# sergioacg/Model-Predictive-Control-Tuning

Hardware: AMD Instinct MI355X
Metric: closed-loop GPC sims/sec (Shell 3x3, N2=30 Nu=5) over tuning grid (higher is better)
Workload: dtype f64; 1 GPU; Shell3x3 GAM scoring: 4096 candidates/GPU x nit=500 closed loop + J1 + RCCL all-gather + ranking; candidates_per_gpu=4096, N2=30, Nu=5, nit=500, parallelism=dp1

## Files before the change

model-predictive-control-tuning_amd/csrc/gpc_kernel.hip:

```cpp
#include <hip/hip_runtime.h>
#include <math.h>

#include "mpct_dev.h"
#include "gi_core.h"
#include "gpc_qp.h"
#include "gpc_qp16.h"
#include "gpc_prologue.h"
#include "gpc_record.h"

namespace mpct {

constexpr int kWaves16 = 3;

struct LdsLayout {
  int rinv, jt, dv, ra, sl, gb, A, x, xc, uprev, yprev, ucum, ye, yeh, uring, mzh, smz, frh, plb, pla, mzb,
      mza, frb, fra, total;
};

__host__ __device__ inline LdsLayout lds_layout(const DevScenario& sc, int M, bool ext) {
  const int nx = sc.nx, nu = sc.nu, nin = sc.nin, ne = sc.ne, my = sc.my;
  const int nmz = sc.dtc ? 2 * my * nu : 0;
  const int nfr = sc.dtc ? my : 0;
  const int ncp = ext ? 2 : 1;
  LdsLayout L;
// ... 428 lines not shown
      st | (nf ? MPCT_ST_NONFINITE_ : 0), iters);
}

}

#include <string>

#include "work_order.h"
#include "launch_fan.h"

namespace mpct {

long long small_lds_bytes(const DevScenario& sc, int M);
int launch_small(const DevScenario& sc, long long C, int nref, const int* N2, const int* Nu, const double* delta,
                 const double* lambda, const double* r, const DevOpts& o, const DevResult& out, const int* perm,
                 int first, hipStream_t stream, std::string* err);
long long dtc_small_lds_bytes(const DevScenario& sc, int M);
int launch_dtc_small(const DevScenario& sc, int cls, long long C, int nref, const int* N2, const int* Nu,
                     const double* delta, const double* lambda, const double* r, const double* v, const DevOpts& o,
                     const DevResult& out, const int* perm, int mlo, int first, hipStream_t stream, std::string* err);

long long lds_bytes_for(const DevScenario& sc, int N2, int Nu, bool ext) {
  (void)N2;
  const int M = sc.nu * Nu;
  if (sc.small && !ext && M <= 16) return small_lds_bytes(sc, M);
  if (sc.small_dtc && !ext && M <= 32) return dtc_small_lds_bytes(sc, M);
  LdsLayout L = lds_layout(sc, M, ext);
  return (long long)L.total * 8;
}

template <int MAXM>
// ... 42 lines not shown
    if (cls <= 32 && sc.small_dtc && !ext) {
      nm += (nm.empty() ? "" : " + ") + std::string("dtc_small_kernel<") + std::to_string(cls) + ">";
      continue;
    }
    if (nm.empty()) nm = "gpc_closed_loop_kernel<" + std::to_string(cls) + tail;
    else if (nm.find("gpc_closed_loop_kernel") == std::string::npos)
      nm += " + gpc_closed_loop_kernel<" + std::to_string(cls) + tail;
    else nm += " + <" + std::to_string(cls) + tail;
  }
  return nm;
}

int launch_closed_loop(const DevScenario& sc, long long C, int nref, const int* N2, const int* Nu,
                       const double* delta, const double* lambda, const double* r,
                       const double* v, const DevOpts& o, const DevResult& out, int maxM,
                       WorkOrder* wo, LaunchFan* fan, hipStream_t stream, std::string* err) {
  if (maxM > 64) {
    *err = "nu*nu_max > 64";
    return -4;
  }
  const int* perm = nullptr;
  DevResult lo = out;
  bool prefilled = false;
  if (wo) {
    if (C >= kOrderMinC) {
      lo.srow = stage_row(out, sc.my, sc.nu);
      const int rs = lo.srow.w ? order_stage(*wo, C * nref, lo.srow.w, &lo.stage, err) : 0;
      if (rs) return rs;
    }
    const int rc = order_candidates(kOrderGpc, sc.my, sc.nu, C, N2, Nu, delta, lambda, *wo, &perm, stream, err,
                                    &sc, nref, r, &lo, &prefilled);
    if (rc) return rc;
  }
  if (!perm) {
    lo = out;
    prefilled = false;
  }
  int rc = prefilled ? 0 : prefill_results(lo, C * nref, sc.my, sc.nu, stream, err);
  if (rc) return rc;
  FanScope fs(top_class(maxM) > 16 ? fan : nullptr, stream);
  int k = 0, mlo = 0;
  for (int cls = 16; cls <= top_class(maxM) && rc == 0; cls *= 2) {
    if (sc.nu > cls) {
      mlo = cls;
      continue;
    }
    const hipStream_t st = fs.stream(k);
    const int first = k == 0;
    const bool ext = o.open_loop || o.want_traj;
    if (diag_drop_launch(k)) rc = 0;
    else if (cls == 16 && sc.small && !ext) rc = launch_small(sc, C, nref, N2, Nu, delta, lambda, r, o, lo, perm, first, st, err);
    else if (cls <= 32 && sc.small_dtc && !ext)
      rc = launch_dtc_small(sc, cls, C, nref, N2, Nu, delta, lambda, r, v, o, lo, perm, mlo, first, st, err);
    else if (cls == 16) rc = launch_t<16>(sc, C, nref, N2, Nu, delta, lambda, r, v, o, lo, perm, mlo, first, st, err);
    else if (cls == 32) rc = launch_t<32>(sc, C, nref, N2, Nu, delta, lambda, r, v, o, lo, perm, mlo, first, st, err);
    else rc = launch_t<64>(sc, C, nref, N2, Nu, delta, lambda, r, v, o, lo, perm, mlo, first, st, err);
    mlo = cls;
    ++k;
  }
  fs.join();
  if (rc == 0 && lo.stage) rc = unpermute_results(*wo, C, nref, sc.my, sc.nu, lo.srow, out, stream, err);
  if (perm) order_mark_used(*wo, stream);
  return rc;
}

}
// ... 1 lines not shown
```

model-predictive-control-tuning_amd/csrc/gpc_qp16.h:

```cpp
#pragma once
#include "gi_core.h"

namespace mpct {

typedef double d4v[4];
#define FOR4(r, ...)             \
  do {                           \
    { constexpr int r = 0; __VA_ARGS__ } \
    { constexpr int r = 1; __VA_ARGS__ } \
    { constexpr int r = 2; __VA_ARGS__ } \
    { constexpr int r = 3; __VA_ARGS__ } \
  } while (0)

struct RegFactors {
  d4v J;
  double* sB;
};
constexpr int kBS = 16;


__device__ __forceinline__ int qlane() {
  int l = threadIdx.x;
  asm volatile("" : "+v"(l));
  return l;
}
__device__ __forceinline__ int q16_i() { return qlane() & 15; }
__device__ __forceinline__ int q16_b() { return qlane() >> 4; }

__device__ __forceinline__ double sel4u_v(double x0, double x1, double x2, double x3, int r) {
  double v = x0;
  if (r == 1) v = x1;
  if (r == 2) v = x2;
  if (r == 3) v = x3;
  return v;
}
#define sel4u(x, r) sel4u_v((x)[0], (x)[1], (x)[2], (x)[3], (r))
__device__ __forceinline__ double sel4v_v(double x0, double x1, double x2, double x3, int r) {
  const double lo = (r & 1) ? x1 : x0;
  const double hi = (r & 1) ? x3 : x2;
  return (r & 2) ? hi : lo;
}
#define sel4v(x, r) sel4v_v((x)[0], (x)[1], (x)[2], (x)[3], (r))

__device__ __forceinline__ void row16_sum4(d4v& t) {
  FOR4(r, t[r] += dppd<kQx1>(t[r]););
  FOR4(r, t[r] += dppd<kQx2>(t[r]););
  FOR4(r, t[r] += dppd<kHalfMirror>(t[r]););
  FOR4(r, t[r] += dppd<kMirror>(t[r]););
}

__device__ __forceinline__ double cvec_at(const d4v& c, int k) {
  return bcast(sel4u(c, k & 3), (k >> 2) * 16);
}

__device__ __forceinline__ void b_row4(const double* sB, d4v& x) {
  const double2* p = reinterpret_cast<const double2*>(sB + q16_i() * kBS + 4 * q16_b());
  const double2 u = p[0], v = p[1];
  x[0] = u.x;
  x[1] = u.y;
  x[2] = v.x;
  x[3] = v.y;
}

__device__ __forceinline__ double rows_down(double v) { return __shfl(v, qlane() + 16, 64); }
__device__ __forceinline__ double rows_up(double v) { return __shfl(v, qlane() - 16, 64); }

__device__ __forceinline__ void rot_pair(double& a, double& c, bool on, double cs, double sn) {
  if (on) {
    const double a0 = a, c0 = c;
    a = cs * a0 + sn * c0;
    c = -sn * a0 + cs * c0;
  }
}
__device__ __forceinline__ void rb_rotate_cols(d4v& x, int jj, double cs, double sn) {
  const int b = q16_b(), b0 = jj >> 2;
  const bool on = b == b0;
  switch (jj & 3) {
    case 0: {
      double a = x[0], c = x[1];
      rot_pair(a, c, on, cs, sn);
      x[0] = a;
      x[1] = c;
      break;
    }
    case 1: {
      double a = x[1], c = x[2];
      rot_pair(a, c, on, cs, sn);
      x[1] = a;
      x[2] = c;
      break;
    }
    case 2: {
      double a = x[2], c = x[3];
      rot_pair(a, c, on, cs, sn);
      x[2] = a;
      x[3] = c;
      break;
    }
    default: {
      const double nx0 = rows_down(x[0]), pv3 = rows_up(x[3]);
      if (on) x[3] = cs * x[3] + sn * nx0;
      if (b == b0 + 1) x[0] = -sn * pv3 + cs * x[0];
      break;
    }
  }
}

struct BoxMark16 {
  template <class St>
  __device__ __forceinline__ void operator()(St& S, int p, bool on) const {
    if (q16_i() == (p >> 2)) {
      if (on) S.act |= 1u << (p & 3);
      else S.act &= ~(1u << (p & 3));
    }
  }
};

template <bool PACKED>
__device__ __forceinline__ int rinv_idx(int i, int k, int M) {
  return PACKED ? i * M - ((i * (i - 1)) >> 1) + (k - i) : i * M + k;
}

template <bool PACKED>
__device__ __forceinline__ void gi16_load_rinv(GIState<16>& S, RegFactors& F, const double* sRi, int M) {
  const int i = q16_i(), b = q16_b();
  FOR4(r, {
    const int k = 4 * b + r;
    F.J[r] = (i < M && k < M && k >= i) ? sRi[rinv_idx<PACKED>(i, k, M)] : 0.0;
  });
  if (i < M) {
    double2* p = reinterpret_cast<double2*>(F.sB + i * kBS + 4 * b);
    p[0] = make_double2(0.0, 0.0);
    p[1] = make_double2(0.0, 0.0);
  }
  S.nrot = 0;
  S.jinit = true;
}

__device__ __forceinline__ void gi16_dvec(const RegFactors& F, int j0, int mp, double sg, d4v& d) {
  const int i = q16_i();
  if (j0 == mp) {
    const int src = j0 + 16 * q16_b();
    FOR4(r, d[r] = __shfl(F.J[r], src, kWave););
  } else {
    const bool in = i >= j0 && i <= mp;
    FOR4(r, d[r] = in ? F.J[r] : 0.0;);
    row16_sum4(d);
  }
  FOR4(r, d[r] *= sg;);
}

__device__ __forceinline__ void gi16_products(const RegFactors& F, const d4v& Bl, const d4v& d, int q,
                                              double& z, double& jq, double& rk, double& dn2, double& beta) {
  const int b = q16_b();
  double za = 0.0, ra = 0.0, s1 = 0.0, s2 = 0.0;
  FOR4(r, {
    const bool tail = 4 * b + r >= q;
    const double d2 = d[r] * d[r];
    s1 += d2;
    if (tail) {
      za = fma(F.J[r], d[r], za);
      s2 += d2;
    } else {
      ra = fma(Bl[r], d[r], ra);
    }
  });
  const double jl = (b == (q >> 2)) ? sel4u(F.J, q & 3) : 0.0;
  z = za;
  jq = jl;
  rk = ra;
  dn2 = s1;
  row4_sum4(z, jq, rk, dn2);
  beta = row4_sum(s2);
}

template <class Mark>
__device__ __forceinline__ void gi16_add(GIState<16>& S, RegFactors& F, double* sRA, int M, int p,
                                         const d4v& d, double beta, double z, double jq, double rk,
                                         double upm, const Mark& mark) {
  const int lane = qlane(), i = lane & 15, b = lane >> 4;
  const int q = S.q;
  const double dq = cvec_at(d, q);
  const double nrm = beta * rsq_nr(beta);
  const double alpha = dq > 0.0 ? -nrm : nrm;
  const double vq = dq - alpha;
  const double two_vtv = qp_rcp(beta - alpha * dq);
  const double f = (z - alpha * jq) * two_vtv;
  const double ia = qp_rcp(alpha);
  FOR4(r, {
    const int k = 4 * b + r;
    if (k >= q) F.J[r] = fma(-f, k == q ? vq : d[r], F.J[r]);
  });
  if (lane <= q) F.sB[lane * kBS + q] = lane < q ? -rk * ia : ia;
  if (lane < q) F.sB[q * kBS + lane] = 0.0;
  {
    const int w = 4 * b + i;
    if (i < 4 && w < q) sRA[w * M + q] = sel4v(d, i);
    if (lane == 0) sRA[q * M + q] = alpha;
  }
  if (i == q) {
    S.uw = upm;
    S.ww = p;
  }
  mark(S, p, true);
  S.q = q + 1;
  S.nrot += 1;
  lds_sync();
}

template <class Mark>
__device__ __forceinline__ void gi16_drop(GIState<16>& S, RegFactors& F, double* sRA, int M, int kd,
                                          const Mark& mark) {
  const int lane = qlane(), i = lane & 15;
  const int q = S.q;
  double* sB = F.sB;
  const int idk = __builtin_amdgcn_readlane(S.ww, kd);
  mark(S, idk, false);
  lds_sync();
  if (lane < q) {
    for (int w = kd; w < q - 1; ++w) {
      sRA[lane * M + w] = sRA[lane * M + w + 1];
      sB[w * kBS + lane] = sB[(w + 1) * kBS + lane];
    }
  }
  {
    const double un = lane_next<16>(S.uw);
    const int wn = lane_next_i<16>(S.ww);
    if (i >= kd && i < q - 1) {
// ... 7 lines not shown
    const double a = sRA[jj * M + jj], c = sRA[(jj + 1) * M + jj];
    const double rr = a * a + c * c;
    if (rr != 0.0) {
      const double ri = rsq_nr(rr);
      const double cs = a * ri, sn = c * ri;
      if (lane >= jj && lane < q - 1) {
        const double r0 = sRA[jj * M + lane], r1 = sRA[(jj + 1) * M + lane];
        sRA[jj * M + lane] = cs * r0 + sn * r1;
        sRA[(jj + 1) * M + lane] = (lane == jj) ? 0.0 : -sn * r0 + cs * r1;
      }
      if (lane < q) {
        const double b0 = sB[lane * kBS + jj], b1 = sB[lane * kBS + jj + 1];
        sB[lane * kBS + jj] = cs * b0 + sn * b1;
        sB[lane * kBS + jj + 1] = -sn * b0 + cs * b1;
      }
      rb_rotate_cols(F.J, jj, cs, sn);
      S.nrot += 1;
    }
    lds_sync();
  }
  const int qn = q - 1;
  if (i == qn) {
    S.uw = 0.0;
    S.ww = -1;
  }
  S.q = qn;
  lds_sync();
}

template <bool PACKED = false, class PAcc = void, bool BLDS = false>
__device__ __forceinline__ int gi_qp16(const double* sRi, double* sRA, int M, int Nu,
                                       const RowCons& rc, double up_row, double xu, double tol, int maxit,
                                       int* st, GIState<16>& S, RegFactors& F, int rebuild, double& xout
#ifdef MPCT_PROFILE
                                       , PAcc& pacc, unsigned long long& pprev
#endif
                                       ) {
  const int lane = qlane(), i = lane & 15;
  const bool row = i < M;
  if (!row) up_row = 0.0;
  const int rl = rc.l;
  double lo_box = 0.0, hi_box = 0.0;
  if constexpr (!BLDS) {
    lo_box = fmax(rc.dmin, rc.umin - up_row);
    hi_box = fmin(rc.dmax, rc.umax - up_row);
  }
  auto slacks = [&](double x, double s[4]) {
    double dmin, dmax, umin, umax, lo, hi;
    if constexpr (BLDS) {
      const double2 a = reinterpret_cast<const double2*>(rc.bnd)[0], b = reinterpret_cast<const double2*>(rc.bnd)[1];
      dmin = a.x;
      dmax = a.y;
      umin = b.x;
// ... 10 lines not shown
    }
    const double pre = block_prefix<16>(x, rl, Nu, row, nullptr);
    if (rl == 0) {
      s[0] = x - lo;
      s[1] = hi - x;
      s[2] = INFINITY;
      s[3] = INFINITY;
    } else {
      s[0] = x - dmin;
      s[1] = dmax - x;
      s[2] = pre - (umin - up_row);
      s[3] = (umax - up_row) - pre;
    }
    if (!row) s[0] = s[1] = s[2] = s[3] = INFINITY;
  };
  const BoxMark16 mark{};
  auto add = [&](int p, const d4v& d, double beta, double z, double jq, double rk, double upm)
                 __attribute__((always_inline)) { gi16_add(S, F, sRA, M, p, d, beta, z, jq, rk, upm, mark); };
  int it = 0;
  double xm = xu;
  PSTAMP(PROF_QCHECK);
  {
    double s[4];
    slacks(xu, s);
    const double smin = fmin(fmin(s[0], s[1]), fmin(s[2], s[3]));
    if (__ballot(smin < -tol) == 0) {
      xout = xu;
      return 0;
    }
    PSTAMP(PROF_QWENTRY);
    if (S.q == 0) {
      S.jinit = false;
    } else {
      if (!S.jinit || S.nrot >= rebuild * M) {
        const int qq = S.q;
#ifdef MPCT_PROFILE
        pacc[PROF_QWREADD] += (unsigned long long)qq * kProfCount;
#endif
        gi16_load_rinv<PACKED>(S, F, sRi, M);
        S.q = 0;
        for (int v = 0; v < qq; ++v) {
          const int p = __builtin_amdgcn_readlane(S.ww, v);
          int j0, mp;
          double sg;
          gi_normal(p, rc, j0, mp, sg);
          d4v Bl, d;
          lds_sync();
          b_row4(F.sB, Bl);
          gi16_dvec(F, j0, mp, sg, d);
          double z, jq, rk, dn2, beta;
          gi16_products(F, Bl, d, v, z, jq, rk, dn2, beta);
          const double uk = S.uw;
          add(p, d, beta, z, jq, rk, 0.0);
          if (i == v) S.uw = uk;
          ++it;
        }
        S.nrot = 0;
      }
      PSTAMP(PROF_QWREB);
      lds_sync();
      double c;
      {
        const int src = (S.ww >= 0 ? S.ww >> 2 : 0) + 16 * q16_b();
        const double g0 = __shfl(s[0], src, kWave), g1 = __shfl(s[1], src, kWave);
        const double g2 = __shfl(s[2], src, kWave), g3 = __shfl(s[3], src, kWave);
        c = i < S.q ? -sel4v_v(g0, g1, g2, g3, S.ww & 3) : 0.0;
      }
      PSTAMP(PROF_QWGATH);
      for (;;) {
        const int q = S.q;
        if (q == 0) {
          xm = xu;
          break;
        }
        d4v Bl, w;
        b_row4(F.sB, Bl);
        FOR4(r, w[r] = i < q ? Bl[r] * c : 0.0;);
        row16_sum4(w);
        const int b = q16_b();
        double xa = 0.0, la = 0.0;
        FOR4(r, {
          if (4 * b + r < q) {
            xa = fma(F.J[r], w[r], xa);
            la = fma(Bl[r], w[r], la);
          }
        });
        row4_sum2(xa, la);
        xm = xu + xa;
        const double lam = la;
        if (i < q) S.uw = lam;
        double lmin = i < q ? lam : INFINITY;
        int kd = i;
        qargmin<16>(lmin, kd, 0);
        PSTAMP(PROF_QWSOLVE);
        if (!(lmin < 0.0)) break;
#ifdef MPCT_PROFILE
        pacc[PROF_QWROT] += (unsigned long long)(S.q - 1 - kd) * kProfCount;
#endif
#ifdef MPCT_DIAG
        if (!(S.diag & kDiagSkipWarmDrop))
#endif
        {
          gi16_drop(S, F, sRA, M, kd, mark);
          {
            const double cn = lane_next<16>(c);
            if (i >= kd && i < q - 1) c = cn;
            else if (i == q - 1) c = 0.0;
          }
        }
        PSTAMP(PROF_QWDROP);
        if (++it >= maxit) {
          *st |= MPCT_ST_QP_MAXITER_;
          break;
        }
      }
      if (!row) xm = 0.0;
    }
  }
// ... 6 lines not shown
      slacks(xm, s);
#pragma unroll
      for (int k = 0; k < 4; ++k)
        if (!((S.act >> k) & 1u) && s[k] < best) {
          best = s[k];
          bid = 4 * i + k;
        }
    }
    qargmin<16>(best, bid, 2);
    PSTAMP(PROF_QCHECK);
    if (!(best < -tol)) break;
    if (it >= maxit) {
      *st |= MPCT_ST_QP_MAXITER_;
      break;
    }
    if (!S.jinit) gi16_load_rinv<PACKED>(S, F, sRi, M);
    const int p = bid;
    int j0, mp;
    double sgp;
    gi_normal(p, rc, j0, mp, sgp);
    double sp = best;
    double upm = 0.0;
    bool infeas = false;
    for (;;) {
      ++it;
      d4v Bl, d;
      b_row4(F.sB, Bl);
      gi16_dvec(F, j0, mp, sgp, d);
      double zm, jq, rk, dn2, beta;
      gi16_products(F, Bl, d, S.q, zm, jq, rk, dn2, beta);
      PSTAMP(PROF_QD);
      double t1 = INFINITY;
      int kdrop = 0x7fffffff;
      if (i < S.q && rk > 0.0) {
        t1 = qp_div(S.uw, rk);
        kdrop = i;
      }
      qargmin<16>(t1, kdrop, 0);
      const double t2 = (beta > 1e-14 * dn2) ? -qp_div(sp, beta) : INFINITY;
      const bool t2inf = __builtin_amdgcn_readfirstlane((int)(t2 == INFINITY)) != 0;
      if (t1 == INFINITY && t2inf) {
        *st |= MPCT_ST_QP_INFEAS_;
        infeas = true;
        break;
      }
// ... 5 lines not shown
      sp += t * beta;
      PSTAMP(PROF_QR);
      if (full) {
        add(p, d, beta, zm, jq, rk, upm);
        PSTAMP(PROF_QADD);
        break;
      }
      if (kdrop >= S.q) {
        *st |= MPCT_ST_NONFINITE_;
        infeas = true;
        break;
      }
#ifdef MPCT_PROFILE
      pacc[PROF_QROT] += (unsigned long long)(S.q - 1 - kdrop) * kProfCount;
#endif
      gi16_drop(S, F, sRA, M, kdrop, mark);
      PSTAMP(PROF_QDROP);
      if (it >= maxit) {
        *st |= MPCT_ST_QP_MAXITER_;
        break;
      }
    }
    if (infeas) break;
  }
  xout = xm;
  return it;
}

}
```

model-predictive-control-tuning_amd/csrc/gpc_small.hip:

```cpp
#include <hip/hip_runtime.h>
#include <math.h>

#include "mpct_dev.h"
#include "gi_core.h"
#include "gpc_qp.h"
#include "gpc_qp16.h"
#include "gpc_prologue.h"
#include "gpc_record.h"

namespace mpct {

struct SmallLayout {
  int rinv, ra, gb, A, xy, ring, hist, bnd, total;
};
__host__ __device__ inline SmallLayout small_layout(const DevScenario& sc, int M) {
  SmallLayout L;
  int o = 0;
  auto take = [&](int n) { int r = o; o += (n + 1) & ~1; return r; };
  L.rinv = take(M * (M + 1) / 2);
  L.ra = take(M * M);
  L.gb = take(M * kBS);
  L.A = take(M * kSmA);
  L.xy = take(kSmY);
  L.ring = take(3 * 2 * kSmR);
  L.hist = take(kSmEOff + 4 * sc.my * sc.sm_ke);
  L.bnd = take(4 * 3);
  L.total = (o + 1) & ~1;
  return L;
}

__device__ __forceinline__ int sm_lane() {
  int l = threadIdx.x;
  asm volatile("" : "+v"(l));
  return l;
}

__global__ void __launch_bounds__(64, 4)
    gpc_small_kernel(const DevScenario sc, long long C, int nref, const int* __restrict__ N2v,
                     const int* __restrict__ Nuv, const double* __restrict__ deltav,
                     const double* __restrict__ lambdav, const double* __restrict__ rv,
                     const int* __restrict__ perm, const DevOpts o, const DevResult out, int first) {
  extern __shared__ __attribute__((aligned(16))) double lds[];
  const int lane = threadIdx.x;
  const long long slot = blockIdx.x;
  const long long S = C * nref;
  if (slot >= S) return;
  const long long cs = slot / nref;
  const int kref = (int)(slot - cs * nref);
  const long long c = perm ? (long long)perm[cs] : cs;
  const long long sim = c * nref + kref;
  const int my = sc.my, nu = sc.nu, nit = sc.nit;
  const int N2 = N2v[c], Nu = Nuv[c];
  const int M = nu * Nu;
  auto write_nan = [&](int status) __attribute__((always_inline)) {
    put_record(out, slot, S, sim, my, nu, lane, NAN, NAN, NAN, NAN, status, 0);
  };
  if (N2 <= 0) {
    if (first) write_nan(MPCT_ST_SKIPPED_);
    return;
  }
  if (N2 > sc.n2max || Nu < 1 || Nu > sc.numax || Nu > N2) {
    if (first) write_nan(MPCT_ST_BADHORIZON_);
    return;
  }
  if (M > 16) return;
// ... 20 lines not shown
  const double pcoef = sc.sm_coef[pv + lane];
  const int pbase = L.hist + sc.sm_hoff[pv + lane];
  const int pc = sc.sm_hc[pv + lane], pmask = sc.sm_hmask[pv + lane];
  const int ke = sc.sm_ke;
  const int oi = (lane >> 2) & 3;
  const int yoff = oi < my ? sc.yoff[oi] : 0;
  const int nyh = oi < my ? sc.nyhi[oi] : 0;
  const int qm = lane & 15, qg = lane >> 4;
  const int aoff = L.A + qm * kSmA + (qg ? kSmY + kSmR * (qg - 1) : 0);
  const int xoff = qg ? L.ring + 2 * kSmR * (qg - 1) : L.xy;
  RowCons rcn;
  rcn.n = qm < M ? qm / Nu : 0;
  rcn.l = qm < M ? qm - rcn.n * Nu : 0;
  if (lane < 4 * nu) lds[L.bnd + lane] = sc.bnd[(lane & 3) * nu + (lane >> 2)];
  rcn.bnd = lds + L.bnd + 4 * rcn.n;
  const double tol = o.feas_tol;
  const int maxit = o.max_qp_iter > 0 ? o.max_qp_iter : 8 * M + 16;
  const int ink0 = sc.ink0;
  const double* rr = rv + (long long)kref * my * nit;
  const int si = oi < my ? oi : my - 1;
  const double* psr = rr + (long long)si * nit;
  const double* psy = sc.yref + (long long)si * nit;
  GIState<16> gis;
  gi_reset<16>(gis);
#ifdef MPCT_DIAG
  gis.diag = o.diag;
#endif
  RegFactors rf;
  FOR4(r, rf.J[r] = 0.0;);
  rf.sB = lds + L.gb;
  long long iters = 0;
  int st = 0;
  double yd0 = 0.0;
  double uprev = 0.0;
  double j1 = 0.0, j22 = 0.0;
  double r_t = psr[0], yr_t = psy[0];
  __builtin_amdgcn_s_waitcnt(0x0F70);

  for (int t = 0; t < nit; ++t) {
    lds_sync();
    const double hv = lds[pbase + ((t - pc) & pmask)];
    const double o1e = lds[L.xy + yoff + 1], o2e = lds[L.xy + yoff + 2];
    const double ye = row4_sum(pcoef * hv);
    double yi = ye + dppd<kQx1>(ye);
    yi += dppd<kQx2>(yi);
    if (sm_lane() < 4 * my) lds[L.hist + kSmEOff + sm_lane() * ke + (t & (ke - 1))] = ye;
    PSTAMP(PROF_PLANT);
    {
      const int l = sm_lane();
      if ((l & ~12) == 0 && (l >> 2) < my) {
        double* xs = lds + L.xy + yoff;
        const double o1 = o1e, o2 = o2e;
        const double n1 = yi - yd0, n2 = n1 - o1, n3 = n2 - o2;
        xs[0] = yi - r_t;
        if (nyh > 1) xs[1] = n1;
        if (nyh > 2) xs[2] = n2;
        if (nyh > 3) xs[3] = n3;
        yd0 = yi;
        const double e1 = yi - yr_t;
        j1 = fma(e1, e1, j1);
        if (t >= ink0) j22 = fma(e1, e1, j22);
      }
    }
    const int tn = t + 1 < nit ? t + 1 : t;
    const double r_n = psr[tn], yr_n = psy[tn];
    lds_sync();
    PSTAMP(PROF_YUPD);
    double xu;
    {
      const int h = (1 - t) & (kSmR - 1);
      const int xo = xoff + (sm_lane() >= 16 ? h : 0);
      const double2* av = reinterpret_cast<const double2*>(lds + aoff);
      const double* xv = lds + xo;
      double a0 = 0.0, a1 = 0.0;
      if ((sm_lane() & 15) < M) {
#pragma unroll
        for (int p = 0; p < kSmR / 2; ++p) {
          const double2 a = av[p];
          a0 = fma(a.x, xv[2 * p], a0);
          a1 = fma(a.y, xv[2 * p + 1], a1);
        }
        if (sm_lane() < 16) {
#pragma unroll
          for (int p = kSmR / 2; p < kSmY / 2; ++p) {
            const double2 a = av[p];
            a0 = fma(a.x, xv[2 * p], a0);
            a1 = fma(a.y, xv[2 * p + 1], a1);
          }
        }
      }
      xu = row4_sum(a0 + a1);
    }
    PSTAMP(PROF_UNC);
    double xq;
    const double up_row = __shfl(uprev, rcn.n, kWave);
    iters += gi_qp16<true, PAccT, true>(lds + L.rinv, lds + L.ra, M, Nu, rcn, up_row, xu, tol, maxit, &st, gis, rf,
                     kGiRebuild16, xq
#ifdef MPCT_PROFILE
                     , pacc, pprev
#endif
    );
    PSTAMP(PROF_QP);
    {
      const int l = sm_lane();
      const double du = __shfl(xq, l < nu ? l * Nu : 0, kWave);
      if (l < nu) {
        const double un = uprev + du;
        uprev = un;
        lds[L.hist + l * kSmU + (t & (kSmU - 1))] = un;
        double* ring = lds + L.ring + 2 * kSmR * l;
        const int p = (-t) & (kSmR - 1);
        ring[p] = du;
        ring[p + kSmR] = du;
      }
    }
    PSTAMP(PROF_UUPD);
    r_t = r_n;
    yr_t = yr_n;
  }
#ifdef MPCT_PROFILE
  if (lane == 0 && out.prof)
    for (int k = 0; k < PROF_N; ++k) out.prof[sim * PROF_N + k] = pacc.get(k);
#endif

  const double j1o = __shfl(j1, (lane & 3) * 4, kWave);
  const double j22o = __shfl(j22, (lane & 3) * 4, kWave);
  if (lane < my && !isfinite(j1o)) st |= MPCT_ST_NONFINITE_;
  const unsigned long long nf = __ballot(st & MPCT_ST_NONFINITE_);
  put_record(out, slot, S, sim, my, nu, lane, j1o, NAN, j22o, NAN, st | (nf ? MPCT_ST_NONFINITE_ : 0), iters);
}

}

#include <string>

namespace mpct {

long long small_lds_bytes(const DevScenario& sc, int M) { return (long long)small_layout(sc, M).total * 8; }

int launch_small(const DevScenario& sc, long long C, int nref, const int* N2, const int* Nu, const double* delta,
                 const double* lambda, const double* r, const DevOpts& o, const DevResult& out, const int* perm,
                 int first, hipStream_t stream, std::string* err) {
  const int nu_cls = sc.numax < 16 / sc.nu ? sc.numax : 16 / sc.nu;
  const long long lds = small_lds_bytes(sc, sc.nu * nu_cls);
  const long long S = C * nref;
  hipLaunchKernelGGL(gpc_small_kernel, dim3((unsigned)S), dim3(kWave), (size_t)lds, stream, sc, C, nref, N2, Nu,
                     delta, lambda, r, perm, o, out, first);
  hipError_t e = hipGetLastError();
  if (e != hipSuccess) {
    *err = std::string("kernel launch failed: ") + hipGetErrorString(e);
    return -3;
  }
  return 0;
}

}
```

model-predictive-control-tuning_amd/csrc/mpct_dev.h:

```cpp
#pragma once
#include <stdint.h>

namespace mpct {

struct WorkOrder {
  void* buf = nullptr;
  size_t bytes = 0;
  const int* perm = nullptr;
  void* stage = nullptr;
  size_t stage_bytes = 0;
  hipEvent_t used = nullptr;
  bool pending = false;
};
constexpr long long kOrderMinC = 256;
constexpr int kGramM = 16;
constexpr int kGramOut = kGramM * kGramM + kGramM;
constexpr long long kGramMaxBytes = 64ll << 20;
constexpr long long kQrtMaxBytes = 16ll << 20;


constexpr int kMaxOut = 16;
constexpr int kMaxIn = 16;
constexpr int kURing = 32;
constexpr int kMaxTaps = 16;
constexpr int kYeHist = 8;
constexpr int kMaxDum = 16;
constexpr int kRegB = 4;
constexpr int kRegA = 4;
constexpr int kRegDu = 8;
// ... 138 lines not shown
```

model-predictive-control-tuning_amd/csrc/mpct_host.cpp:

```cpp
#include <hip/hip_runtime.h>

#include <algorithm>
#include <cmath>
#include <cstring>
#include <string>
#include <vector>
#include <cstdio>
#include <thread>

#include "scenario_tables.h"
#include "launch_fan.h"
#include "work_order.h"
#include "dtc_robust.h"
#include "pareto.h"
#include "hv_select.h"
#include "hypervolume.h"
#include "hypervolume_exact.h"
#include "traj_indices.h"
#include "draw_stats.h"

namespace mpct {
int launch_closed_loop(const DevScenario& sc, long long C, int nref, const int* N2, const int* Nu,
                       const double* delta, const double* lambda, const double* r,
                       const double* v, const DevOpts& o, const DevResult& out, int maxM,
                       WorkOrder* wo, LaunchFan* fan, hipStream_t stream, std::string* err);
long long lds_bytes_for(const DevScenario& sc, int N2, int Nu, bool ext);
std::string closed_loop_instance(const DevScenario& sc, int maxM, bool ext);
int launch_mdband(const DevScenario& sc, long long C, int nref, const int* N2, const int* Nu, const double* delta,
                  const double* lambda, const double* r, const double* v, const DevOpts& o, const DevResult& out,
                  hipStream_t stream, LaunchFan* fan, std::string* err);
long long mdband_lds_bytes(const DevScenario& sc, int N2, int Nu, int ncopy);
int launch_nmpc(const DevScenario& sc, long long C, int nref, const int* N, const int* Nu, const double* delta,
                const double* lambda, const double* r, const DevOpts& o, const DevResult& out, hipStream_t stream,
                LaunchFan* fan, WorkOrder* wo, std::string* err);
long long nmpc_lds_bytes(int M, int N);
}

using namespace mpct;

struct DevCtx {
// ... 21 lines not shown

static thread_local std::string g_err;

static int fail(int code, const std::string& msg) {
  g_err = msg;
  return code;
}

extern "C" int32_t mpct_abi_version(void) { return MPCT_ABI_VERSION; }
extern "C" const char* mpct_last_error(void) { return g_err.c_str(); }

static int32_t created(std::unique_ptr<mpct_scenario> s, const BuildError& err, mpct_scenario** out) {
  if (!s) return fail(err.code, err.msg);
  const char* e = getenv("MPCT_NO_QR_TABLES");
  if (e && *e && atoi(e) != 0) s->qr_tables = 0;
  *out = s.release();
  g_err.clear();
  return MPCT_OK;
}

extern "C" int32_t mpct_scenario_create(const mpct_scenario_desc* d, mpct_scenario** out) {
  if (!d || !out) return fail(MPCT_EINVAL, "null argument");
  *out = nullptr;
  BuildError err;
  return created(build_scenario(*d, &err), err, out);
}

extern "C" int32_t mpct_scenario_create_est(const mpct_scenario_desc* d, int32_t estimator, mpct_scenario** out) {
  if (!d || !out) return fail(MPCT_EINVAL, "null argument");
  *out = nullptr;
// ... 183 lines not shown
  unsigned long long* dprof = nullptr;
  (void)hipMalloc(&dprof, sizeof(unsigned long long) * S * 4);
  (void)hipMemset(dprof, 0, sizeof(unsigned long long) * S * 4);
  dr.prof = dprof;
#endif
  std::string err;
  int rc = 0;
  if (dop.want_traj)
    rc = fill_unrun_trajectories(dr, C, nref, N2, Nu, cx->ds.n2max, cx->ds.numax, s->my, s->nu, s->nit,
                                 dop.open_loop != 0, stream, &err);
  if (rc) return fail(rc, err);
  if (s->nmpc)
    rc = launch_nmpc(cx->ds, C, nref, N2, Nu, delta, lambda, r, dop, dr, stream, &cx->fan, &cx->order, &err);
  else if (s->mdband)
    rc = launch_mdband(cx->ds, C, nref, N2, Nu, delta, lambda, r, v, dop, dr, stream, &cx->fan, &err);
  else
    rc = launch_closed_loop(cx->ds, C, nref, N2, Nu, delta, lambda, r, v, dop, dr, s->nu * s->numax, &cx->order, &cx->fan,
                            stream, &err);
  if (rc) return fail(rc, err);
#ifdef MPCT_TIMELINE
  {
    std::vector<unsigned long long> hp(S * 4);
    (void)hipStreamSynchronize(stream);
    (void)hipMemcpy(hp.data(), dprof, sizeof(unsigned long long) * S * 4, hipMemcpyDeviceToHost);
    (void)hipFree(dprof);
    const char* path = getenv("MPCT_TIMELINE_OUT");
    if (path) {
      FILE* f = fopen(path, "wb");
      if (f) {
        fwrite(hp.data(), sizeof(unsigned long long), hp.size(), f);
        fclose(f);
      }
    }
// ... 1599 lines not shown
```

model-predictive-control-tuning_amd/csrc/scenario_tables.h:

```cpp
#pragma once
#include <hip/hip_runtime.h>

#include <algorithm>
#include <cmath>
#include <cstring>
#include <memory>
#include <string>
#include <vector>

#include "../../include/mpct.h"
#include "mpct_dev.h"

struct DevCtx;

namespace mpct {
struct ZTables {
  int maxb = 0, maxa = 0;
  std::vector<int> nb, na, off;
  std::vector<double> b, a;
};
}

struct mpct_scenario {
  int my = 0, nu = 0, nd = 0, nin = 0, nit = 0, n2max = 0, numax = 0, wsq = 1, ink0 = 9;
// ... 15 lines not shown
  std::vector<int> fr_n;
  std::vector<double> bnd;
  std::vector<double> yref;
  int mdband = 0;
  int est = 0;
  double rho = 0.0;
  std::vector<double> step_md;
  std::vector<double> obnd;
  std::vector<double> wscale;
  int nmpc = 0, nsub = 10, sqp_max = 100;
  double ts = 0.0, sqp_tol = 1e-8;
  std::vector<int> xc;
  std::vector<double> nm;
  std::vector<double> nmv;
  int qr_tables = 1;
  std::vector<DevCtx*> ctx;
  std::vector<std::vector<DevCtx*>> extra;
};

namespace mpct {

struct BuildError {
  int code = MPCT_OK;
  std::string msg;
};
struct Rejected {
  operator std::unique_ptr<mpct_scenario>() const { return nullptr; }
  operator bool() const { return false; }
};
inline Rejected reject(BuildError* err, int code, const char* msg) {
// ... 806 lines not shown
```

Baseline: 2.195 million sims/s.

## Split small GPC kernel into register-heavy wide variant and normal variant on concurrent streams

Adds a second instantiation of the small GPC kernel with lower occupancy (launch bounds 64,2). It keeps the A-row coefficients and box bounds in registers instead of LDS and drops the asm lane barriers. A slot-splitting rule based on CU count sends part of the simulation slots to the wide kernel and the rest to the normal kernel on an auxiliary fan stream, so the two run concurrently. The aim is to cut LDS traffic and fill the device better when the slot count is near 16×CU. The cost is higher register pressure and extra stream and launch complexity.

```diff
diff --git a/model-predictive-control-tuning_amd/csrc/gpc_kernel.hip b/model-predictive-control-tuning_amd/csrc/gpc_kernel.hip
--- a/model-predictive-control-tuning_amd/csrc/gpc_kernel.hip
+++ b/model-predictive-control-tuning_amd/csrc/gpc_kernel.hip
@@ -466,7 +466,7 @@
 long long small_lds_bytes(const DevScenario& sc, int M);
 int launch_small(const DevScenario& sc, long long C, int nref, const int* N2, const int* Nu, const double* delta,
                  const double* lambda, const double* r, const DevOpts& o, const DevResult& out, const int* perm,
-                 int first, hipStream_t stream, std::string* err);
+                 int first, long long slot0, long long nslot, bool wide, hipStream_t stream, std::string* err);
 long long dtc_small_lds_bytes(const DevScenario& sc, int M);
 int launch_dtc_small(const DevScenario& sc, int cls, long long C, int nref, const int* N2, const int* Nu,
                      const double* delta, const double* lambda, const double* r, const double* v, const DevOpts& o,
@@ -539,7 +539,7 @@
 int launch_closed_loop(const DevScenario& sc, long long C, int nref, const int* N2, const int* Nu,
                        const double* delta, const double* lambda, const double* r,
                        const double* v, const DevOpts& o, const DevResult& out, int maxM,
-                       WorkOrder* wo, LaunchFan* fan, hipStream_t stream, std::string* err) {
+                       WorkOrder* wo, LaunchFan* fan, long long wide, int ncu, hipStream_t stream, std::string* err) {
   if (maxM > 64) {
     *err = "nu*nu_max > 64";
     return -4;
@@ -563,7 +563,11 @@
   }
   int rc = prefilled ? 0 : prefill_results(lo, C * nref, sc.my, sc.nu, stream, err);
   if (rc) return rc;
-  FanScope fs(top_class(maxM) > 16 ? fan : nullptr, stream);
+  const bool ext = o.open_loop || o.want_traj;
+  const long long S = C * nref;
+  long long H = wide_slots(S, ncu, perm && sc.small && !ext && sc.nu <= 16 && fan && fan->ready, wide);
+  FanScope fs(top_class(maxM) > 16 || H > 0 ? fan : nullptr, stream);
+  if (!fs.fan) H = 0;
   int k = 0, mlo = 0;
   for (int cls = 16; cls <= top_class(maxM) && rc == 0; cls *= 2) {
     if (sc.nu > cls) {
@@ -572,9 +576,13 @@
     }
     const hipStream_t st = fs.stream(k);
     const int first = k == 0;
-    const bool ext = o.open_loop || o.want_traj;
     if (diag_drop_launch(k)) rc = 0;
-    else if (cls == 16 && sc.small && !ext) rc = launch_small(sc, C, nref, N2, Nu, delta, lambda, r, o, lo, perm, first, st, err);
+    else if (cls == 16 && sc.small && !ext) {
+      if (H > 0) rc = launch_small(sc, C, nref, N2, Nu, delta, lambda, r, o, lo, perm, first, 0, H, true, st, err);
+      if (rc == 0 && H < S)
+        rc = launch_small(sc, C, nref, N2, Nu, delta, lambda, r, o, lo, perm, first, H, S - H, false,
+                          H > 0 ? fs.stream(kFanAux) : st, err);
+    }
     else if (cls <= 32 && sc.small_dtc && !ext)
       rc = launch_dtc_small(sc, cls, C, nref, N2, Nu, delta, lambda, r, v, o, lo, perm, mlo, first, st, err);
     else if (cls == 16) rc = launch_t<16>(sc, C, nref, N2, Nu, delta, lambda, r, v, o, lo, perm, mlo, first, st, err);
diff --git a/model-predictive-control-tuning_amd/csrc/gpc_qp16.h b/model-predictive-control-tuning_amd/csrc/gpc_qp16.h
--- a/model-predictive-control-tuning_amd/csrc/gpc_qp16.h
+++ b/model-predictive-control-tuning_amd/csrc/gpc_qp16.h
@@ -19,13 +19,16 @@
 constexpr int kBS = 16;
 
 
+template <bool W = false>
 __device__ __forceinline__ int qlane() {
   int l = threadIdx.x;
-  asm volatile("" : "+v"(l));
+  if constexpr (!W) asm volatile("" : "+v"(l));
   return l;
 }
-__device__ __forceinline__ int q16_i() { return qlane() & 15; }
-__device__ __forceinline__ int q16_b() { return qlane() >> 4; }
+template <bool W = false>
+__device__ __forceinline__ int q16_i() { return qlane<W>() & 15; }
+template <bool W = false>
+__device__ __forceinline__ int q16_b() { return qlane<W>() >> 4; }
 
 __device__ __forceinline__ double sel4u_v(double x0, double x1, double x2, double x3, int r) {
   double v = x0;
@@ -53,8 +56,9 @@
   return bcast(sel4u(c, k & 3), (k >> 2) * 16);
 }
 
+template <bool W = false>
 __device__ __forceinline__ void b_row4(const double* sB, d4v& x) {
-  const double2* p = reinterpret_cast<const double2*>(sB + q16_i() * kBS + 4 * q16_b());
+  const double2* p = reinterpret_cast<const double2*>(sB + q16_i<W>() * kBS + 4 * q16_b<W>());
   const double2 u = p[0], v = p[1];
   x[0] = u.x;
   x[1] = u.y;
@@ -62,8 +66,10 @@
   x[3] = v.y;
 }
 
-__device__ __forceinline__ double rows_down(double v) { return __shfl(v, qlane() + 16, 64); }
-__device__ __forceinline__ double rows_up(double v) { return __shfl(v, qlane() - 16, 64); }
+template <bool W = false>
+__device__ __forceinline__ double rows_down(double v) { return __shfl(v, qlane<W>() + 16, 64); }
+template <bool W = false>
+__device__ __forceinline__ double rows_up(double v) { return __shfl(v, qlane<W>() - 16, 64); }
 
 __device__ __forceinline__ void rot_pair(double& a, double& c, bool on, double cs, double sn) {
   if (on) {
@@ -72,8 +78,9 @@
     c = -sn * a0 + cs * c0;
   }
 }
+template <bool W = false>
 __device__ __forceinline__ void rb_rotate_cols(d4v& x, int jj, double cs, double sn) {
-  const int b = q16_b(), b0 = jj >> 2;
+  const int b = q16_b<W>(), b0 = jj >> 2;
   const bool on = b == b0;
   switch (jj & 3) {
     case 0: {
@@ -98,7 +105,7 @@
       break;
     }
     default: {
-      const double nx0 = rows_down(x[0]), pv3 = rows_up(x[3]);
+      const double nx0 = rows_down<W>(x[0]), pv3 = rows_up<W>(x[3]);
       if (on) x[3] = cs * x[3] + sn * nx0;
       if (b == b0 + 1) x[0] = -sn * pv3 + cs * x[0];
       break;
@@ -106,24 +113,26 @@
   }
 }
 
-struct BoxMark16 {
+template <bool W>
+struct BoxMark16T {
   template <class St>
   __device__ __forceinline__ void operator()(St& S, int p, bool on) const {
-    if (q16_i() == (p >> 2)) {
+    if (q16_i<W>() == (p >> 2)) {
       if (on) S.act |= 1u << (p & 3);
       else S.act &= ~(1u << (p & 3));
     }
   }
 };
+using BoxMark16 = BoxMark16T<false>;
 
 template <bool PACKED>
 __device__ __forceinline__ int rinv_idx(int i, int k, int M) {
   return PACKED ? i * M - ((i * (i - 1)) >> 1) + (k - i) : i * M + k;
 }
 
-template <bool PACKED>
+template <bool PACKED, bool W = false>
 __device__ __forceinline__ void gi16_load_rinv(GIState<16>& S, RegFactors& F, const double* sRi, int M) {
-  const int i = q16_i(), b = q16_b();
+  const int i = q16_i<W>(), b = q16_b<W>();
   FOR4(r, {
     const int k = 4 * b + r;
     F.J[r] = (i < M && k < M && k >= i) ? sRi[rinv_idx<PACKED>(i, k, M)] : 0.0;
@@ -137,10 +146,11 @@
   S.jinit = true;
 }
 
+template <bool W = false>
 __device__ __forceinline__ void gi16_dvec(const RegFactors& F, int j0, int mp, double sg, d4v& d) {
-  const int i = q16_i();
+  const int i = q16_i<W>();
   if (j0 == mp) {
-    const int src = j0 + 16 * q16_b();
+    const int src = j0 + 16 * q16_b<W>();
     FOR4(r, d[r] = __shfl(F.J[r], src, kWave););
   } else {
     const bool in = i >= j0 && i <= mp;
@@ -150,9 +160,10 @@
   FOR4(r, d[r] *= sg;);
 }
 
+template <bool W = false>
 __device__ __forceinline__ void gi16_products(const RegFactors& F, const d4v& Bl, const d4v& d, int q,
                                               double& z, double& jq, double& rk, double& dn2, double& beta) {
-  const int b = q16_b();
+  const int b = q16_b<W>();
   double za = 0.0, ra = 0.0, s1 = 0.0, s2 = 0.0;
   FOR4(r, {
     const bool tail = 4 * b + r >= q;
@@ -174,11 +185,11 @@
   beta = row4_sum(s2);
 }
 
-template <class Mark>
+template <bool W = false, class Mark>
 __device__ __forceinline__ void gi16_add(GIState<16>& S, RegFactors& F, double* sRA, int M, int p,
                                          const d4v& d, double beta, double z, double jq, double rk,
                                          double upm, const Mark& mark) {
-  const int lane = qlane(), i = lane & 15, b = lane >> 4;
+  const int lane = qlane<W>(), i = lane & 15, b = lane >> 4;
   const int q = S.q;
   const double dq = cvec_at(d, q);
   const double nrm = beta * rsq_nr(beta);
@@ -208,10 +219,10 @@
   lds_sync();
 }
 
-template <class Mark>
+template <bool W = false, class Mark>
 __device__ __forceinline__ void gi16_drop(GIState<16>& S, RegFactors& F, double* sRA, int M, int kd,
                                           const Mark& mark) {
-  const int lane = qlane(), i = lane & 15;
+  const int lane = qlane<W>(), i = lane & 15;
   const int q = S.q;
   double* sB = F.sB;
   const int idk = __builtin_amdgcn_readlane(S.ww, kd);
@@ -249,7 +260,7 @@
         sB[lane * kBS + jj] = cs * b0 + sn * b1;
         sB[lane * kBS + jj + 1] = -sn * b0 + cs * b1;
       }
-      rb_rotate_cols(F.J, jj, cs, sn);
+      rb_rotate_cols<W>(F.J, jj, cs, sn);
       S.nrot += 1;
     }
     lds_sync();
@@ -263,7 +274,7 @@
   lds_sync();
 }
 
-template <bool PACKED = false, class PAcc = void, bool BLDS = false>
+template <bool PACKED = false, class PAcc = void, bool BLDS = false, bool W = false>
 __device__ __forceinline__ int gi_qp16(const double* sRi, double* sRA, int M, int Nu,
                                        const RowCons& rc, double up_row, double xu, double tol, int maxit,
                                        int* st, GIState<16>& S, RegFactors& F, int rebuild, double& xout
@@ -271,7 +282,7 @@
                                        , PAcc& pacc, unsigned long long& pprev
 #endif
                                        ) {
-  const int lane = qlane(), i = lane & 15;
+  const int lane = qlane<W>(), i = lane & 15;
   const bool row = i < M;
   if (!row) up_row = 0.0;
   const int rl = rc.l;
@@ -312,9 +323,9 @@
     }
     if (!row) s[0] = s[1] = s[2] = s[3] = INFINITY;
   };
-  const BoxMark16 mark{};
+  const BoxMark16T<W> mark{};
   auto add = [&](int p, const d4v& d, double beta, double z, double jq, double rk, double upm)
-                 __attribute__((always_inline)) { gi16_add(S, F, sRA, M, p, d, beta, z, jq, rk, upm, mark); };
+                 __attribute__((always_inline)) { gi16_add<W>(S, F, sRA, M, p, d, beta, z, jq, rk, upm, mark); };
   int it = 0;
   double xm = xu;
   PSTAMP(PROF_QCHECK);
@@ -335,7 +346,7 @@
 #ifdef MPCT_PROFILE
         pacc[PROF_QWREADD] += (unsigned long long)qq * kProfCount;
 #endif
-        gi16_load_rinv<PACKED>(S, F, sRi, M);
+        gi16_load_rinv<PACKED, W>(S, F, sRi, M);
         S.q = 0;
         for (int v = 0; v < qq; ++v) {
           const int p = __builtin_amdgcn_readlane(S.ww, v);
@@ -344,10 +355,10 @@
           gi_normal(p, rc, j0, mp, sg);
           d4v Bl, d;
           lds_sync();
-          b_row4(F.sB, Bl);
-          gi16_dvec(F, j0, mp, sg, d);
+          b_row4<W>(F.sB, Bl);
+          gi16_dvec<W>(F, j0, mp, sg, d);
           double z, jq, rk, dn2, beta;
-          gi16_products(F, Bl, d, v, z, jq, rk, dn2, beta);
+          gi16_products<W>(F, Bl, d, v, z, jq, rk, dn2, beta);
           const double uk = S.uw;
           add(p, d, beta, z, jq, rk, 0.0);
           if (i == v) S.uw = uk;
@@ -359,7 +370,7 @@
       lds_sync();
       double c;
       {
-        const int src = (S.ww >= 0 ? S.ww >> 2 : 0) + 16 * q16_b();
+        const int src = (S.ww >= 0 ? S.ww >> 2 : 0) + 16 * q16_b<W>();
         const double g0 = __shfl(s[0], src, kWave), g1 = __shfl(s[1], src, kWave);
         const double g2 = __shfl(s[2], src, kWave), g3 = __shfl(s[3], src, kWave);
         c = i < S.q ? -sel4v_v(g0, g1, g2, g3, S.ww & 3) : 0.0;
@@ -372,10 +383,10 @@
           break;
         }
         d4v Bl, w;
-        b_row4(F.sB, Bl);
+        b_row4<W>(F.sB, Bl);
         FOR4(r, w[r] = i < q ? Bl[r] * c : 0.0;);
         row16_sum4(w);
-        const int b = q16_b();
+        const int b = q16_b<W>();
         double xa = 0.0, la = 0.0;
         FOR4(r, {
           if (4 * b + r < q) {
@@ -399,7 +410,7 @@
         if (!(S.diag & kDiagSkipWarmDrop))
 #endif
         {
-          gi16_drop(S, F, sRA, M, kd, mark);
+          gi16_drop<W>(S, F, sRA, M, kd, mark);
           {
             const double cn = lane_next<16>(c);
             if (i >= kd && i < q - 1) c = cn;
@@ -436,7 +447,7 @@
       *st |= MPCT_ST_QP_MAXITER_;
       break;
     }
-    if (!S.jinit) gi16_load_rinv<PACKED>(S, F, sRi, M);
+    if (!S.jinit) gi16_load_rinv<PACKED, W>(S, F, sRi, M);
     const int p = bid;
     int j0, mp;
     double sgp;
@@ -447,10 +458,10 @@
     for (;;) {
       ++it;
       d4v Bl, d;
-      b_row4(F.sB, Bl);
-      gi16_dvec(F, j0, mp, sgp, d);
+      b_row4<W>(F.sB, Bl);
+      gi16_dvec<W>(F, j0, mp, sgp, d);
       double zm, jq, rk, dn2, beta;
-      gi16_products(F, Bl, d, S.q, zm, jq, rk, dn2, beta);
+      gi16_products<W>(F, Bl, d, S.q, zm, jq, rk, dn2, beta);
       PSTAMP(PROF_QD);
       double t1 = INFINITY;
       int kdrop = 0x7fffffff;
@@ -486,7 +497,7 @@
 #ifdef MPCT_PROFILE
       pacc[PROF_QROT] += (unsigned long long)(S.q - 1 - kdrop) * kProfCount;
 #endif
-      gi16_drop(S, F, sRA, M, kdrop, mark);
+      gi16_drop<W>(S, F, sRA, M, kdrop, mark);
       PSTAMP(PROF_QDROP);
       if (it >= maxit) {
         *st |= MPCT_ST_QP_MAXITER_;
diff --git a/model-predictive-control-tuning_amd/csrc/gpc_small.hip b/model-predictive-control-tuning_amd/csrc/gpc_small.hip
--- a/model-predictive-control-tuning_amd/csrc/gpc_small.hip
+++ b/model-predictive-control-tuning_amd/csrc/gpc_small.hip
@@ -7,6 +7,20 @@
 #include "gpc_qp16.h"
 #include "gpc_prologue.h"
 #include "gpc_record.h"
+
+#ifndef MPCT_WIDE_BREG
+#define MPCT_WIDE_BREG 1
+#endif
+#ifndef MPCT_WIDE_AREG
+#define MPCT_WIDE_AREG 1
+#endif
+#ifndef MPCT_WIDE_PLAIN
+#ifdef MPCT_DIAG
+#define MPCT_WIDE_PLAIN 0
+#else
+#define MPCT_WIDE_PLAIN 1
+#endif
+#endif
 
 namespace mpct {
 
@@ -29,26 +43,30 @@
   return L;
 }
 
+template <bool WIDE>
 __device__ __forceinline__ int sm_lane() {
   int l = threadIdx.x;
-  asm volatile("" : "+v"(l));
+  if constexpr (!WIDE) asm volatile("" : "+v"(l));
   return l;
 }
 
-__global__ void __launch_bounds__(64, 4)
-    gpc_small_kernel(const DevScenario sc, long long C, int nref, const int* __restrict__ N2v,
+template <bool WIDE>
+__device__ __forceinline__ void gpc_small_body(const DevScenario& sc, long long C, int nref, const int* __restrict__ N2v,
                      const int* __restrict__ Nuv, const double* __restrict__ deltav,
                      const double* __restrict__ lambdav, const double* __restrict__ rv,
-                     const int* __restrict__ perm, const DevOpts o, const DevResult out, int first) {
+                     const int* __restrict__ perm, const DevOpts& o, const DevResult& out, int first,
+                     long long slot0, long long nslot) {
   extern __shared__ __attribute__((aligned(16))) double lds[];
   const int lane = threadIdx.x;
-  const long long slot = blockIdx.x;
   const long long S = C * nref;
+  if ((long long)blockIdx.x >= nslot) return;
+  const long long slot = slot0 + blockIdx.x;
   if (slot >= S) return;
   const long long cs = slot / nref;
   const int kref = (int)(slot - cs * nref);
   const long long c = perm ? (long long)perm[cs] : cs;
   const long long sim = c * nref + kref;
+  constexpr bool kWideBReg = WIDE && MPCT_WIDE_BREG, kWideAReg = WIDE && MPCT_WIDE_AREG, kPlain = WIDE && MPCT_WIDE_PLAIN;
   const int my = sc.my, nu = sc.nu, nit = sc.nit;
   const int N2 = N2v[c], Nu = Nuv[c];
   const int M = nu * Nu;
@@ -99,6 +117,12 @@
   rcn.l = qm < M ? qm - rcn.n * Nu : 0;
   if (lane < 4 * nu) lds[L.bnd + lane] = sc.bnd[(lane & 3) * nu + (lane >> 2)];
   rcn.bnd = lds + L.bnd + 4 * rcn.n;
+  if constexpr (kWideBReg) {
+    rcn.dmin = sc.bnd[0 * nu + rcn.n];
+    rcn.dmax = sc.bnd[1 * nu + rcn.n];
+    rcn.umin = sc.bnd[2 * nu + rcn.n];
+    rcn.umax = sc.bnd[3 * nu + rcn.n];
+  }
   const double tol = o.feas_tol;
   const int maxit = o.max_qp_iter > 0 ? o.max_qp_iter : 8 * M + 16;
   const int ink0 = sc.ink0;
@@ -120,6 +144,20 @@
   double uprev = 0.0;
   double j1 = 0.0, j22 = 0.0;
   double r_t = psr[0], yr_t = psy[0];
+  double ar[kSmY];
+#pragma unroll
+  for (int p = 0; p < kSmY; ++p) ar[p] = 0.0;
+  if constexpr (kWideAReg) {
+    lds_sync();
+    if (qm < M) {
+#pragma unroll
+      for (int p = 0; p < kSmR; ++p) ar[p] = lds[aoff + p];
+      if (lane < 16) {
+#pragma unroll
+        for (int p = kSmR; p < kSmY; ++p) ar[p] = lds[aoff + p];
+      }
+    }
+  }
   __builtin_amdgcn_s_waitcnt(0x0F70);
 
   for (int t = 0; t < nit; ++t) {
@@ -129,10 +167,10 @@
     const double ye = row4_sum(pcoef * hv);
     double yi = ye + dppd<kQx1>(ye);
     yi += dppd<kQx2>(yi);
-    if (sm_lane() < 4 * my) lds[L.hist + kSmEOff + sm_lane() * ke + (t & (ke - 1))] = ye;
+    if (sm_lane<kPlain>() < 4 * my) lds[L.hist + kSmEOff + sm_lane<kPlain>() * ke + (t & (ke - 1))] = ye;
     PSTAMP(PROF_PLANT);
     {
-      const int l = sm_lane();
+      const int l = sm_lane<kPlain>();
       if ((l & ~12) == 0 && (l >> 2) < my) {
         double* xs = lds + L.xy + yoff;
         const double o1 = o1e, o2 = o2e;
@@ -154,18 +192,33 @@
     double xu;
     {
       const int h = (1 - t) & (kSmR - 1);
-      const int xo = xoff + (sm_lane() >= 16 ? h : 0);
+      const int xo = xoff + (sm_lane<kPlain>() >= 16 ? h : 0);
       const double2* av = reinterpret_cast<const double2*>(lds + aoff);
       const double* xv = lds + xo;
       double a0 = 0.0, a1 = 0.0;
-      if ((sm_lane() & 15) < M) {
+      if constexpr (kWideAReg) {
+        if (qm < M) {
+#pragma unroll
+          for (int p = 0; p < kSmR / 2; ++p) {
+            a0 = fma(ar[2 * p], xv[2 * p], a0);
+            a1 = fma(ar[2 * p + 1], xv[2 * p + 1], a1);
+          }
+          if (lane < 16) {
+#pragma unroll
+            for (int p = kSmR / 2; p < kSmY / 2; ++p) {
+              a0 = fma(ar[2 * p], xv[2 * p], a0);
+              a1 = fma(ar[2 * p + 1], xv[2 * p + 1], a1);
+            }
+          }
+        }
+      } else if ((sm_lane<kPlain>() & 15) < M) {
 #pragma unroll
         for (int p = 0; p < kSmR / 2; ++p) {
           const double2 a = av[p];
           a0 = fma(a.x, xv[2 * p], a0);
           a1 = fma(a.y, xv[2 * p + 1], a1);
         }
-        if (sm_lane() < 16) {
+        if (sm_lane<kPlain>() < 16) {
 #pragma unroll
           for (int p = kSmR / 2; p < kSmY / 2; ++p) {
             const double2 a = av[p];
@@ -179,7 +232,7 @@
     PSTAMP(PROF_UNC);
     double xq;
     const double up_row = __shfl(uprev, rcn.n, kWave);
-    iters += gi_qp16<true, PAccT, true>(lds + L.rinv, lds + L.ra, M, Nu, rcn, up_row, xu, tol, maxit, &st, gis, rf,
+    iters += gi_qp16<true, PAccT, !kWideBReg, kPlain>(lds + L.rinv, lds + L.ra, M, Nu, rcn, up_row, xu, tol, maxit, &st, gis, rf,
                      kGiRebuild16, xq
 #ifdef MPCT_PROFILE
                      , pacc, pprev
@@ -187,7 +240,7 @@
     );
     PSTAMP(PROF_QP);
     {
-      const int l = sm_lane();
+      const int l = sm_lane<kPlain>();
       const double du = __shfl(xq, l < nu ? l * Nu : 0, kWave);
       if (l < nu) {
         const double un = uprev + du;
@@ -215,6 +268,24 @@
   put_record(out, slot, S, sim, my, nu, lane, j1o, NAN, j22o, NAN, st | (nf ? MPCT_ST_NONFINITE_ : 0), iters);
 }
 
+__global__ void __launch_bounds__(64, 4)
+    gpc_small_kernel(const DevScenario sc, long long C, int nref, const int* __restrict__ N2v,
+                     const int* __restrict__ Nuv, const double* __restrict__ deltav,
+                     const double* __restrict__ lambdav, const double* __restrict__ rv,
+                     const int* __restrict__ perm, const DevOpts o, const DevResult out, int first,
+                     long long slot0, long long nslot) {
+  gpc_small_body<false>(sc, C, nref, N2v, Nuv, deltav, lambdav, rv, perm, o, out, first, slot0, nslot);
+}
+
+__global__ void __launch_bounds__(64, 2)
+    gpc_small_wide_kernel(const DevScenario sc, long long C, int nref, const int* __restrict__ N2v,
+                          const int* __restrict__ Nuv, const double* __restrict__ deltav,
+                          const double* __restrict__ lambdav, const double* __restrict__ rv,
+                          const int* __restrict__ perm, const DevOpts o, const DevResult out, int first,
+                          long long slot0, long long nslot) {
+  gpc_small_body<true>(sc, C, nref, N2v, Nuv, deltav, lambdav, rv, perm, o, out, first, slot0, nslot);
+}
+
 }
 
 #include <string>
@@ -225,12 +296,12 @@
 
 int launch_small(const DevScenario& sc, long long C, int nref, const int* N2, const int* Nu, const double* delta,
                  const double* lambda, const double* r, const DevOpts& o, const DevResult& out, const int* perm,
-                 int first, hipStream_t stream, std::string* err) {
+                 int first, long long slot0, long long nslot, bool wide, hipStream_t stream, std::string* err) {
   const int nu_cls = sc.numax < 16 / sc.nu ? sc.numax : 16 / sc.nu;
   const long long lds = small_lds_bytes(sc, sc.nu * nu_cls);
-  const long long S = C * nref;
-  hipLaunchKernelGGL(gpc_small_kernel, dim3((unsigned)S), dim3(kWave), (size_t)lds, stream, sc, C, nref, N2, Nu,
-                     delta, lambda, r, perm, o, out, first);
+  if (nslot <= 0) return 0;
+  hipLaunchKernelGGL(wide ? gpc_small_wide_kernel : gpc_small_kernel, dim3((unsigned)nslot), dim3(kWave), (size_t)lds,
+                     stream, sc, C, nref, N2, Nu, delta, lambda, r, perm, o, out, first, slot0, nslot);
   hipError_t e = hipGetLastError();
   if (e != hipSuccess) {
     *err = std::string("kernel launch failed: ") + hipGetErrorString(e);
diff --git a/model-predictive-control-tuning_amd/csrc/mpct_dev.h b/model-predictive-control-tuning_amd/csrc/mpct_dev.h
--- a/model-predictive-control-tuning_amd/csrc/mpct_dev.h
+++ b/model-predictive-control-tuning_amd/csrc/mpct_dev.h
@@ -13,6 +13,18 @@
   bool pending = false;
 };
 constexpr long long kOrderMinC = 256;
+
+inline long long wide_slot_rule(long long S, int ncu) {
+  const long long cap = 16LL * ncu;
+  if (ncu <= 0 || S < kOrderMinC || S > cap) return 0;
+  if (2 * S <= cap) return S;
+  return cap - S > cap / 4 ? cap - S : cap / 4;
+}
+inline long long wide_slots(long long S, int ncu, bool eligible, long long forced) {
+  if (!eligible) return 0;
+  const long long h = forced >= 0 ? forced : wide_slot_rule(S, ncu);
+  return h < S ? h : S;
+}
 constexpr int kGramM = 16;
 constexpr int kGramOut = kGramM * kGramM + kGramM;
 constexpr long long kGramMaxBytes = 64ll << 20;
diff --git a/model-predictive-control-tuning_amd/csrc/mpct_host.cpp b/model-predictive-control-tuning_amd/csrc/mpct_host.cpp
--- a/model-predictive-control-tuning_amd/csrc/mpct_host.cpp
+++ b/model-predictive-control-tuning_amd/csrc/mpct_host.cpp
@@ -23,7 +23,7 @@
 int launch_closed_loop(const DevScenario& sc, long long C, int nref, const int* N2, const int* Nu,
                        const double* delta, const double* lambda, const double* r,
                        const double* v, const DevOpts& o, const DevResult& out, int maxM,
-                       WorkOrder* wo, LaunchFan* fan, hipStream_t stream, std::string* err);
+                       WorkOrder* wo, LaunchFan* fan, long long wide, int ncu, hipStream_t stream, std::string* err);
 long long lds_bytes_for(const DevScenario& sc, int N2, int Nu, bool ext);
 std::string closed_loop_instance(const DevScenario& sc, int maxM, bool ext);
 int launch_mdband(const DevScenario& sc, long long C, int nref, const int* N2, const int* Nu, const double* delta,
@@ -75,6 +75,8 @@
   if (!s) return fail(err.code, err.msg);
   const char* e = getenv("MPCT_NO_QR_TABLES");
   if (e && *e && atoi(e) != 0) s->qr_tables = 0;
+  const char* w = getenv("MPCT_WIDE_SLOTS");
+  if (w && *w && atoll(w) >= 0) s->wide_slots = atoll(w);
   *out = s.release();
   g_err.clear();
   return MPCT_OK;
@@ -288,9 +290,13 @@
     rc = launch_nmpc(cx->ds, C, nref, N2, Nu, delta, lambda, r, dop, dr, stream, &cx->fan, &cx->order, &err);
   else if (s->mdband)
     rc = launch_mdband(cx->ds, C, nref, N2, Nu, delta, lambda, r, v, dop, dr, stream, &cx->fan, &err);
-  else
+  else {
+    if (cx->ncu == 0 &&
+        (hipDeviceGetAttribute(&cx->ncu, hipDeviceAttributeMultiprocessorCount, cx->dev) != hipSuccess || cx->ncu < 1))
+      cx->ncu = 0;
     rc = launch_closed_loop(cx->ds, C, nref, N2, Nu, delta, lambda, r, v, dop, dr, s->nu * s->numax, &cx->order, &cx->fan,
-                            stream, &err);
+                            s->wide_slots, cx->ncu, stream, &err);
+  }
   if (rc) return fail(rc, err);
 #ifdef MPCT_TIMELINE
   {
diff --git a/model-predictive-control-tuning_amd/csrc/scenario_tables.h b/model-predictive-control-tuning_amd/csrc/scenario_tables.h
--- a/model-predictive-control-tuning_amd/csrc/scenario_tables.h
+++ b/model-predictive-control-tuning_amd/csrc/scenario_tables.h
@@ -53,6 +53,7 @@
   std::vector<double> nm;
   std::vector<double> nmv;
   int qr_tables = 1;
+  long long wide_slots = -1;
   std::vector<DevCtx*> ctx;
   std::vector<std::vector<DevCtx*>> extra;
 };
```

After: 2.329 million sims/s, median of 6. 1.06x the previous value.
